# songlab-cal/CherryML

Hardware: AMD Instinct MI355X
Metric: cherry-pairs/sec (whole node) per EM iter (higher is better)
Workload: dtype f64

## Files before the change

cherryml_amd/csrc/eigh_planned.hip.h:

```cpp
#pragma once
#include "jacobi_block.hip.h"
#include "large_bank.hip.h"

enum {
  EC_STALL = 0,
  EC_FINAL = 1,
  EC_NSWEEP = 2,
  EC_MODE = 3,
  EC_SQ = 4,
  EC_ERR = 5,
  EC_ARRIVE = 6,
  EC_MASKED = 7,
  EC_SC = 8,
  EC_BANDS = 9,
  EC_SIGMA = 10,
  EC_TBSTALE = 11,
  EC_SKIP = 12,
  EC_REC = 16,
  EC_MAXREC = 12,
  EC_JSTATE = 64,
  EC_T0 = 80,
  EC_TSWEEP = 81,
  EC_TEND = 93,
  EC_NSTAMP = 95,
  EC_STAMPS = 96,
#ifdef CB_EIGH_STAMPS
  EC_WORDS = 96 + 96
#else
  EC_WORDS = 96
#endif
};
#ifdef CB_EIGH_STAMPS
__device__ __forceinline__ void lge_stamp(unsigned long long *ctl, int id) {
  if (blockIdx.x == 0 && blockIdx.y == 0 && threadIdx.x == 0) {
    const unsigned long long i = atomicAdd(ctl + EC_NSTAMP, 1ull);
    if (i < 96ull) ctl[EC_STAMPS + i] = ((unsigned long long)__builtin_amdgcn_s_memrealtime() << 8) | (unsigned long long)id;
  }
}
#define LGE_STAMP(ctl, id) lge_stamp(const_cast<unsigned long long *>(ctl), id)
#else

#define LGE_STAMP(ctl, id) ((void)0)
#endif
#define EC_NONE 0xFFFFFFFFull
#ifdef CB_PLAIN_WORDS
typedef const unsigned long long *lge_const_words;
#else
typedef const __attribute__((address_space(4))) unsigned long long *lge_const_words;
#endif

struct GramArgs {
  int LD, band, slot;
  int cap;
  int nsq;
  const double *G;
  double *X, *Xf;
  double *Gm, *dg;
  int so;
  unsigned long long *acc;
  unsigned long long *ctl;
  double trigger;
};

#define LGE_ACC_NT 32
#define LGE_ACC_COS 64
#define LGE_ACC_WORDS 128
#define LGE_ACC_UNIT 4503599627370496.0
__device__ __forceinline__ unsigned long long lge_fix(double x) {
  return x > 0.0 ? (unsigned long long)(fmin(x, 16.0) * LGE_ACC_UNIT) + 1ull : 0ull;
}

struct DecArgs {
  int on = 0;
  int cap = 0, nsq = 0, so = 0;
  double trigger = 0.0;
  const unsigned long long *acc = nullptr;
};

__device__ __forceinline__ double lge_lim(int order) {
  return order == 2 ? 1e-5 : order == 4 ? 2e-3 : order == 8 ? 0.06 : 0.5;
}

__global__ __launch_bounds__(512, 6) void lge_gram(GramArgs a) {
  __shared__ double sRed[8][256];
  __shared__ double sDg[2][32][16];
  __shared__ double sD[2][16];
  __shared__ double sStat[3][4];
  const unsigned long long *ctl = a.ctl;
  LGE_STAMP(ctl, 4);
  {
    lge_const_words cw = (lge_const_words)ctl;
    const unsigned long long w_stall = cw[EC_STALL], w_final = cw[EC_FINAL];
    if (w_stall != 0ull || (unsigned long long)a.slot > w_final) return;
  }
  const int LD = a.LD, nt = LD / 16;
  const int tm = blockIdx.x / nt, tn = blockIdx.x - tm * nt;
  const int m0 = tm * 16, n0 = tn * 16;
  const int wave = threadIdx.x >> 6, lane = threadIdx.x & 63, lo = lane & 15, hi = lane >> 4;
  const double *rowA = a.G + (size_t)(m0 + lo) * LD + 4 * hi, *rowB = a.G + (size_t)(n0 + lo) * LD + 4 * hi;
  d4 acc0 = {0.0, 0.0, 0.0, 0.0}, acc1 = acc0;
  double da = 0.0, db = 0.0;
  const int nchunks = LD / 16;
  for (int j0 = wave; j0 < nchunks; j0 += 32) {
    d4 av[4], bv[4];
#pragma unroll
    for (int u = 0; u < 4; ++u) {
      const int j = min(j0 + 8 * u, nchunks - 1);
      av[u] = *reinterpret_cast<const d4 *>(rowA + 16 * j);
      bv[u] = *reinterpret_cast<const d4 *>(rowB + 16 * j);
    }
#pragma unroll
    for (int u = 0; u < 4; ++u) {
      if (j0 + 8 * u < nchunks) {
        acc0 = mfma_f64(av[u][0], bv[u][0], acc0);
        acc1 = mfma_f64(av[u][1], bv[u][1], acc1);
        acc0 = mfma_f64(av[u][2], bv[u][2], acc0);
        acc1 = mfma_f64(av[u][3], bv[u][3], acc1);
        da += (av[u][0] * av[u][0] + av[u][1] * av[u][1]) + (av[u][2] * av[u][2] + av[u][3] * av[u][3]);
        db += (bv[u][0] * bv[u][0] + bv[u][1] * bv[u][1]) + (bv[u][2] * bv[u][2] + bv[u][3] * bv[u][3]);
      }
    }
  }
  const d4 acc = acc0 + acc1;
#pragma unroll
  for (int r = 0; r < 4; ++r) sRed[wave][r * 64 + lane] = acc[r];
  sDg[0][wave * 4 + hi][lo] = da;
  sDg[1][wave * 4 + hi][lo] = db;
  __syncthreads();
  if (threadIdx.x < 32) {
    const int w = threadIdx.x >> 4, c = threadIdx.x & 15;
    double s0 = 0.0, s1 = 0.0, s2 = 0.0, s3 = 0.0;
#pragma unroll
    for (int p = 0; p < 32; p += 4) {
      s0 += sDg[w][p][c];
      s1 += sDg[w][p + 1][c];
      s2 += sDg[w][p + 2][c];
      s3 += sDg[w][p + 3][c];
    }
    sD[w][c] = (s0 + s1) + (s2 + s3);
  }
  __syncthreads();
  double mc2 = 0.0;
  if (threadIdx.x < 256) {
    const int t = threadIdx.x, r = t >> 6, l = t & 63;
    const int ri = (l >> 4) + 4 * r, ci = l & 15;
    const int row = m0 + ri, col = n0 + ci;
    double g = 0.0;
#pragma unroll
    for (int w = 0; w < 8; ++w) g += sRed[w][t];
    const double gii = sD[0][ri], gjj = sD[1][ci];
    double x = 0.0;
    const double g2 = g * g, ab = gii * gjj;
    if (!(g2 == g2) || !(ab == ab)) mc2 = INFINITY;
    if (row != col && g2 > ab * (CB_JAC_SKIP * CB_JAC_SKIP)) {
      mc2 = fmax(mc2, g2 * fast_rcp(ab));
      const double d = gjj - gii;
      x = d != 0.0 ? 0.5 * atan(2.0 * g * fast_rcp(d)) : (g > 0.0 ? 0.78539816339744831 : -0.78539816339744831);
    }
    const int bd = row / JB_W - col / JB_W;
    const bool far = bd > a.band || -bd > a.band;
    a.X[(size_t)row * LD + col] = x;
    a.Xf[(size_t)row * LD + col] = far ? x : 0.0;
    if (a.so) {
      a.Gm[(size_t)row * LD + col] = g;
      if (row == col) a.dg[row] = gii;
    }
    double rs = fabs(x), rsf = far ? fabs(x) : 0.0;
#pragma unroll
    for (int m = 1; m < 16; m <<= 1) {
      rs += __shfl_xor(rs, m);
      rsf += __shfl_xor(rsf, m);
      mc2 = fmax(mc2, __shfl_xor(mc2, m));
    }
#pragma unroll
    for (int m = 16; m < 64; m <<= 1) {
      rs = fmax(rs, __shfl_xor(rs, m));
      rsf = fmax(rsf, __shfl_xor(rsf, m));
      mc2 = fmax(mc2, __shfl_xor(mc2, m));
    }
    if (l == 0) {
      sStat[0][r] = rs;
      sStat[1][r] = rsf;
      sStat[2][r] = mc2;
    }
  }
  __syncthreads();
  if (threadIdx.x < 3) {
    const int k = threadIdx.x;
    const double v = fmax(fmax(sStat[k][0], sStat[k][1]), fmax(sStat[k][2], sStat[k][3]));
    if (k < 2) atomicAdd(a.acc + k * LGE_ACC_NT + tm, lge_fix(v));
    else atomicMax(a.acc + LGE_ACC_COS + 16 * (blockIdx.x & 3), dbl_bits(v));
  }
}

struct LgeDecision {
  unsigned long long mode, sq, sc_bits;
};
struct LgeAcc {
  unsigned long long w = 0ull, c2 = 0ull;
};
__device__ __forceinline__ LgeAcc lge_acc_request(const DecArgs &d) {
  LgeAcc q;
  if (d.on) {
    q.w = d.acc[threadIdx.x & 63];
    lge_const_words ar = (lge_const_words)d.acc;
#pragma unroll
    for (int i = 0; i < 4; ++i) {
      const unsigned long long c = ar[LGE_ACC_COS + 16 * i];
      q.c2 = c > q.c2 ? c : q.c2;
    }
  }
  return q;
}
__device__ __forceinline__ double lge_uniform(double v, int lane) {
  return __hiloint2double(__builtin_amdgcn_readlane(__double2hiint(v), lane), __builtin_amdgcn_readlane(__double2loint(v), lane));
}
__device__ __forceinline__ LgeDecision lge_decide_here(int slot, const DecArgs &d, const LgeAcc &q, unsigned long long *ctl,
                                                       unsigned long long nsweep) {
  double v = (double)q.w * (1.0 / LGE_ACC_UNIT);
#pragma unroll
  for (int m = 1; m < 32; m <<= 1) v = fmax(v, __shfl_xor(v, m));
  const double rowsum = lge_uniform(v, 0), rowsum_far = lge_uniform(v, 32);
  double c2;
  memcpy(&c2, &q.c2, 8);
  LgeDecision o{0ull, 0ull, 0x3FF0000000000000ull};
  const bool bad = q.c2 >= 0x7FF0000000000000ull;
  bool masked = false, fin = false;
  if (!bad) {
    masked = c2 > d.trigger * d.trigger || rowsum > 1.0;
    const double rsu = masked ? rowsum_far : rowsum;
    const bool so = d.so != 0 && !masked && c2 > 1e-16 && rowsum <= 0.3;
    const double r2 = rowsum * rowsum;
    fin = !masked && (c2 <= 1e-16 || (so && c2 * r2 * r2 <= 4e-28));
    int order = rsu <= lge_lim(2) ? 2 : rsu <= lge_lim(4) ? 4 : rsu <= lge_lim(8) ? 8 : 12;
    if (order > d.cap) order = d.cap;
    const double lim = lge_lim(order);
    double sc = 1.0;
    while (rsu * sc > lim) {
      sc *= 0.5;
      ++o.sq;
    }
    unsigned long long damped = 0ull;
    if (o.sq > (unsigned long long)d.nsq) {
      o.sq = (unsigned long long)d.nsq;
      sc = lim / rsu;
      damped = 1ull;
    }
    o.sc_bits = dbl_bits(sc);
    o.mode = (unsigned long long)order | (masked ? 256ull : 0ull) | (damped << 9) | (so ? 1024ull : 0ull) | (1ull << 16);
  }
  if (blockIdx.x == 0 && blockIdx.y == 0 && threadIdx.x == 0) {
    const unsigned long long k = nsweep;
    ctl[EC_NSWEEP] = k + 1;
    if (bad) {
      ctl[EC_ERR] = 2ull;
      ctl[EC_STALL] = 1ull;
    }
    if (fin) ctl[EC_FINAL] = (unsigned long long)slot;
    ctl[EC_MASKED] = masked ? 1ull : 0ull;
    ctl[EC_MODE] = o.mode;
    ctl[EC_SQ] = o.sq;
    ctl[EC_SC] = o.sc_bits;
    if (k < EC_MAXREC) {
      ctl[EC_TSWEEP + k] = __builtin_amdgcn_s_memrealtime();
      ctl[EC_REC + 4 * k + 0] = dbl_bits(sqrt(c2));
      ctl[EC_REC + 4 * k + 1] = dbl_bits(rowsum);
      ctl[EC_REC + 4 * k + 2] = dbl_bits(rowsum_far);
      ctl[EC_REC + 4 * k + 3] = o.mode | (o.sq << 24) | ((unsigned long long)slot << 32);
    }
  }
  return o;
}

#ifdef CB_DECIDE_KERNEL
__global__ void lge_decide_k(int slot, DecArgs d, unsigned long long *ctl) {
  const LgeAcc q = lge_acc_request(d);
  lge_const_words cw = (lge_const_words)ctl;
  const unsigned long long w_stall = cw[EC_STALL], w_final = cw[EC_FINAL], w_nsw = cw[EC_NSWEEP];
  if (w_stall != 0ull || (unsigned long long)slot > w_final) return;
  (void)lge_decide_here(slot, d, q, ctl, w_nsw);
}
#endif

#ifdef CB_NANCHECK
__global__ void lge_residual(int LD, const double *A, const double *Ut, const double *lam, unsigned long long *ctl) {
  const int k = blockIdx.x;
  double m = 0.0;
  for (int i = threadIdx.x; i < LD; i += blockDim.x) {
    double r = -lam[k] * Ut[(size_t)k * LD + i];
    for (int j = 0; j < LD; ++j) r = fma(A[(size_t)i * LD + j], Ut[(size_t)k * LD + j], r);
    m = fmax(m, fabs(r));
    if (!(r == r)) m = INFINITY;
  }
  m = wave_max(m);
  if ((threadIdx.x & 63) == 0) atomicMax(ctl + 92, dbl_bits(m));
}
#endif
#ifdef CB_NANCHECK
__global__ void lge_orthcheck(int LD, const double *R, unsigned long long slot, unsigned long long *ctl) {
  lge_const_words cw = (lge_const_words)ctl;
  if (cw[EC_STALL] != 0ull || slot > cw[EC_FINAL] || !(cw[EC_MODE] >> 16)) return;
  const int k = blockIdx.x;
  double m = 0.0;
  for (int j = threadIdx.x; j < LD; j += blockDim.x) {
    double d = j == k ? -1.0 : 0.0;
    for (int i = 0; i < LD; ++i) d = fma(R[(size_t)i * LD + k], R[(size_t)i * LD + j], d);
    m = fmax(m, fabs(d));
    if (!(d == d)) m = INFINITY;
  }
  m = wave_max(m);
  if ((threadIdx.x & 63) == 0) {
    const unsigned long long old = atomicMax(ctl + 91, dbl_bits(m));
    if (dbl_bits(m) > old) ctl[90] = slot;
  }
}
#endif
#ifdef CB_NANCHECK
__global__ void lge_nancheck(int LD, const double *buf, unsigned long long tag, unsigned long long *ctl) {
  const size_t i = (size_t)blockIdx.x * blockDim.x + threadIdx.x;
  if (i >= (size_t)LD * LD) return;
  const double v = buf[i];
  if (!(v - v == 0.0)) atomicCAS(ctl + 94, 0ull, tag);
}
#endif

enum { EG_P2 = 0, EG_P34, EG_T1, EG_RP, EG_SQ, EG_GR, EG_R4 };

struct EgArgs {
  int LD, slot, kind, q;
  int cap;
  int early;
  const unsigned long long *ctl;
  const double *X, *Xf;
  double *P2, *P4;
  double *B0, *B1, *B2;
  double *T;
  double *R[2], *Rt[2];
  double *Rfin;
  const double *Gin;
  double *Gout;
  DecArgs dec;
  unsigned long long *zacc;
};


__device__ __forceinline__ double lge_ld(const double *base, int s, int LD, int c0, unsigned lane_bytes) {
  const __amdgpu_buffer_rsrc_t rs = __builtin_amdgcn_make_buffer_rsrc(const_cast<double *>(base), 0, 0x7fffffff, 0x00027000);
  return __builtin_bit_cast(double, __builtin_amdgcn_raw_buffer_load_b64(rs, (int)lane_bytes, (int)((unsigned)(4 * s * LD + c0) * 8u), 0));
}

__device__ __forceinline__ double lge_fold8(double (*sRed)[256], d4 acc, int wave, int lane, int et) {
  if (wave >= 4) {
#pragma unroll
    for (int r = 0; r < 4; ++r) sRed[wave - 4][r * 64 + lane] = acc[r];
  }
  __syncthreads();
  if (wave < 4) {
#pragma unroll
    for (int r = 0; r < 4; ++r) acc[r] += sRed[wave][r * 64 + lane];
  }
  __syncthreads();
  if (wave < 4) {
#pragma unroll
    for (int r = 0; r < 4; ++r) sRed[wave][r * 64 + lane] = acc[r];
  }
  __syncthreads();
  return (sRed[0][et] + sRed[1][et]) + (sRed[2][et] + sRed[3][et]);
}

#define LGE_UU 13
template <int KIND>
__global__ __launch_bounds__(512) void lge_gemm(EgArgs a) {
  __shared__ double sRed[4][256];
  const unsigned long long *ctl = a.ctl;
  LGE_STAMP(ctl, 10 + KIND);
  const int LD = a.LD, nt = LD / 16;
  const int tm = blockIdx.x / nt, tn = blockIdx.x - tm * nt;
  const int m0 = tm * 16, n0 = tn * 16;
  const int wave = __builtin_amdgcn_readfirstlane(threadIdx.x >> 6), lane = threadIdx.x & 63, lo = lane & 15, hi = lane >> 4;
  const int nsteps = LD / 4;
  const unsigned loff = (unsigned)(hi * LD + lo) * 8u;
  const int et = threadIdx.x & 255, er = et >> 6, el = et & 63;
  const int row = m0 + (el >> 4) + 4 * er, col = n0 + (el & 15);
  const size_t idx = (size_t)row * LD + col;
  const bool ep = threadIdx.x < 256;
  const double *Ap = nullptr, *Bp = nullptr, *Ep = nullptr;
  if (KIND == EG_T1) { Ap = a.P4; Bp = a.B2; Ep = a.B1; }
  if (KIND == EG_RP) { Ap = a.P4; Bp = a.T; Ep = a.B0; }
  if (KIND == EG_SQ) { Ap = a.Rt[a.q & 1]; Bp = a.R[a.q & 1]; }
  if (KIND == EG_GR) { Ap = a.Rfin; Bp = a.Gin; }
  if (KIND == EG_R4) { Ap = a.P2; Bp = a.B0; Ep = a.P2; }
  double av[LGE_UU], bv[LGE_UU], e1 = 0.0, ex = 0.0;
  const bool early = KIND != EG_P2 && a.early != 0;
  if (early) {
#pragma unroll
    for (int u = 0; u < LGE_UU; ++u) {
      const int sk = min(wave + 8 * u, nsteps - 1);
      av[u] = lge_ld(Ap, sk, LD, m0, loff);
      bv[u] = lge_ld(Bp, sk, LD, n0, loff);
    }
    if (Ep && ep) e1 = Ep[idx];
  }
  LgeAcc accq;
  if (KIND == EG_P2) accq = lge_acc_request(a.dec);
  lge_const_words cw = (lge_const_words)ctl;
  const unsigned long long w_stall = cw[EC_STALL], w_final = cw[EC_FINAL], w_nsw = cw[EC_NSWEEP];
  unsigned long long mode = cw[EC_MODE], w_sq = cw[EC_SQ], w_sc = cw[EC_SC];
  if (w_stall != 0ull || (unsigned long long)a.slot > w_final) return;
  if (KIND == EG_P2 && a.dec.on) {
    const LgeDecision dd = lge_decide_here(a.slot, a.dec, accq, const_cast<unsigned long long *>(ctl), w_nsw);
    mode = dd.mode;
    w_sq = dd.sq;
    w_sc = dd.sc_bits;
  }
  if (!(mode >> 16)) return;
  if (KIND == EG_GR && a.zacc && blockIdx.x == 0 && threadIdx.x < LGE_ACC_WORDS)
    a.zacc[threadIdx.x] = 0ull;
  const int order = (int)(mode & 255ull);
  const bool masked = (mode & (256ull | 1024ull)) != 0ull;
  const int sq = (int)w_sq;
  double sc;
  memcpy(&sc, &w_sc, 8);
  const double *Xu = masked ? a.Xf : a.X;
  if (KIND == EG_R4 && order != 4) return;
  if (KIND == EG_T1 && order != 12) return;
  if (KIND == EG_RP && order < 8) return;
  if (KIND == EG_SQ && a.q >= sq) return;
  if (!early) {
    const double *pa = KIND == EG_P2 ? Xu : Ap, *pb = KIND == EG_P2 ? Xu : Bp;
#pragma unroll
    for (int u = 0; u < LGE_UU; ++u) {
      const int sk = min(wave + 8 * u, nsteps - 1);
      av[u] = lge_ld(pa, sk, LD, m0, loff);
      bv[u] = lge_ld(pb, sk, LD, n0, loff);
    }
    if (KIND != EG_P2 && Ep && ep) e1 = Ep[idx];
  }
  if ((KIND == EG_P2 || KIND == EG_R4) && ep) ex = Xu[idx];
  d4 acc = {0.0, 0.0, 0.0, 0.0};
#pragma unroll
  for (int u = 0; u < LGE_UU; ++u)
    if (wave + 8 * u < nsteps) acc = mfma_f64(av[u], bv[u], acc);
  for (int s0 = wave + 8 * LGE_UU; s0 < nsteps; s0 += 8 * LGE_UU) {
    const double *pa = KIND == EG_P2 ? Xu : Ap, *pb = KIND == EG_P2 ? Xu : Bp;
#pragma unroll
    for (int u = 0; u < LGE_UU; ++u) {
      const int sk = min(s0 + 8 * u, nsteps - 1);
      av[u] = lge_ld(pa, sk, LD, m0, loff);
      bv[u] = lge_ld(pb, sk, LD, n0, loff);
    }
#pragma unroll
    for (int u = 0; u < LGE_UU; ++u)
      if (s0 + 8 * u < nsteps) acc = mfma_f64(av[u], bv[u], acc);
  }
  const double v = lge_fold8(sRed, acc, wave, lane, et);
  if (!ep) return;
  const double edl = row == col ? 1.0 : 0.0, s2 = sc * sc;
  if (KIND == EG_P2) {
    if (order == 2) {
      a.Rfin[idx] = fma(-0.5 * s2, v, fma(sc, ex, edl));
    } else {
      a.P2[idx] = v;
      if (a.cap == 4) a.B0[idx] = fma(-s2 * (1.0 / 24.0), v, (sc * (1.0 / 6.0)) * ex);
    }
  } else if (KIND == EG_R4) {
    a.Rfin[idx] = fma(-s2, v, fma(-0.5 * s2, e1, fma(sc, ex, edl)));
  } else if (KIND == EG_T1) {
    a.T[idx] = fma(s2 * s2, v, e1);
  } else if (KIND == EG_RP) {
    const double o = fma(s2 * s2, v, e1);
    if (sq == 0) a.Rfin[idx] = o;
    else {
      a.R[0][idx] = o;
      a.Rt[0][(size_t)col * LD + row] = o;
    }
  } else if (KIND == EG_SQ) {
    if (a.q == sq - 1) a.Rfin[idx] = v;
    else {
      a.R[(a.q + 1) & 1][idx] = v;
      a.Rt[(a.q + 1) & 1][(size_t)col * LD + row] = v;
    }
  } else {
    a.Gout[idx] = v;
  }
}

__global__ __launch_bounds__(512) void lge_p34(EgArgs a) {
  __shared__ double sRed[8][256];
  const unsigned long long *ctl = a.ctl;
  LGE_STAMP(ctl, 17);
  const int LD = a.LD, nt = LD / 16;
  const int tm = blockIdx.x / nt, tn = blockIdx.x - tm * nt;
  const int m0 = tm * 16, n0 = tn * 16;
  const int wave = __builtin_amdgcn_readfirstlane(threadIdx.x >> 6), lane = threadIdx.x & 63, lo = lane & 15, hi = lane >> 4;
  const int w4 = wave & 3;
  const bool fourth = wave >= 4;
  const int nsteps = LD / 4;
  const unsigned loff = (unsigned)(hi * LD + lo) * 8u;
  const int et = threadIdx.x & 255, er = et >> 6, el = et & 63;
  const int row = m0 + (el >> 4) + 4 * er, col = n0 + (el & 15);
  const size_t idx = (size_t)row * LD + col;
  const bool ep = threadIdx.x < 256;
  double av[LGE_UU], bv[LGE_UU], e2 = 0.0;
  const bool early = a.early != 0;
  if (early) {
#pragma unroll
    for (int u = 0; u < LGE_UU; ++u) {
      const int sk = min(w4 + 4 * u, nsteps - 1);
      bv[u] = lge_ld(a.P2, sk, LD, n0, loff);
      if (fourth) av[u] = lge_ld(a.P2, sk, LD, m0, loff);
    }
    if (ep) e2 = a.P2[idx];
  }
  lge_const_words cw = (lge_const_words)ctl;
  const unsigned long long w_stall = cw[EC_STALL], w_final = cw[EC_FINAL], mode = cw[EC_MODE], w_sc = cw[EC_SC];
  if (w_stall != 0ull || (unsigned long long)a.slot > w_final) return;
  if (!(mode >> 16)) return;
  const int order = (int)(mode & 255ull);
  if (order < 4) return;
  const bool masked = (mode & (256ull | 1024ull)) != 0ull;
  double sc;
  memcpy(&sc, &w_sc, 8);
  const double *Xu = masked ? a.Xf : a.X;
  const double *Ap = fourth ? a.P2 : Xu;
  if (!early) {
#pragma unroll
    for (int u = 0; u < LGE_UU; ++u) {
      const int sk = min(w4 + 4 * u, nsteps - 1);
      bv[u] = lge_ld(a.P2, sk, LD, n0, loff);
      av[u] = lge_ld(Ap, sk, LD, m0, loff);
    }
    if (ep) e2 = a.P2[idx];
  } else if (!fourth) {
#pragma unroll
    for (int u = 0; u < LGE_UU; ++u) av[u] = lge_ld(Xu, min(w4 + 4 * u, nsteps - 1), LD, m0, loff);
  }
  double ex = 0.0;
  if (ep) ex = Xu[idx];
  d4 acc = {0.0, 0.0, 0.0, 0.0};
#pragma unroll
  for (int u = 0; u < LGE_UU; ++u)
    if (w4 + 4 * u < nsteps) acc = mfma_f64(av[u], bv[u], acc);
  for (int s0 = w4 + 4 * LGE_UU; s0 < nsteps; s0 += 4 * LGE_UU) {
#pragma unroll
    for (int u = 0; u < LGE_UU; ++u) {
      const int sk = min(s0 + 4 * u, nsteps - 1);
// ... 277 lines not shown
```

cherryml_amd/csrc/eigh_planned_host.hip.h:

```cpp
#pragma once

struct EighRecord {
  bool stall = false;
  int err = 0, nsweep = 0, final_slot = -1;
  double sigma = 0.0;
  bool tb_stale = false;
  struct {
    double c, rs, rsf;
    int order, sq, slot;
    bool masked, damped;
  } sweep[EC_MAXREC];
};

#ifndef CB_PLANNED_BAND
#define CB_PLANNED_BAND 1
#endif
#ifndef CB_LEAD_INNER
#define CB_LEAD_INNER 2
#endif
static const int kPlannedBand = CB_PLANNED_BAND;

static void eigh_plan_default(EighPlan &p, int extra = 0) {
  p = EighPlan{};
  p.lead_band = 1;
// ... 33 lines not shown
  }
  p.slot[n] = EighSlot{4, 0, 0, 1, 0, 2, 0};
  p.lead_band = (r.sweep[0].masked && r.sweep[0].c > 1e-3) ? 1 : 0;
}

static void eigh_plan_continue(const EighRecord &r, EighPlan &p) {
  eigh_plan_default(p, 0);
  const bool masked = r.nsweep > 0 && r.sweep[std::min(r.nsweep, (int)EC_MAXREC) - 1].masked;
  p.lead_band = masked ? 1 : 0;
}

static bool eigh_planned_setup(cb_bank *h) {
  if (h->ectl) return true;
  if (h->planned_unavailable) return false;
  if (h->LD / 16 > LGE_ACC_NT) return false;
  h->planned_unavailable = true;
  const int LD = h->LD;
  void *q = nullptr;
  if (hipMalloc(&q, EC_WORDS * sizeof(unsigned long long)) != hipSuccess) return false;
  h->allocs.push_back(q);
  unsigned long long *ctl = static_cast<unsigned long long *>(q);
  if (hipMalloc(&q, ((size_t)2 * LGE_ACC_WORDS + LD) * sizeof(double)) != hipSuccess) return false;
  h->allocs.push_back(q);
  h->epart = static_cast<double *>(q);
  if (!h->epin) {
    if (hipHostMalloc(&q, 2 * (EC_WORDS + 16) * sizeof(unsigned long long), hipHostMallocCoherent | hipHostMallocMapped) != hipSuccess) {
      (void)hipGetLastError();
      return false;
    }
    memset(q, 0, 2 * (EC_WORDS + 16) * sizeof(unsigned long long));
    h->epin = static_cast<unsigned long long *>(q);
  }
  const int RS = LD + ((2 - LD % 32 + 32) % 32);
  const size_t lds = (size_t)(16 * RS + 3 * 16 * 17 + JB_WAVES * 256) * sizeof(double);
  if (hipFuncSetAttribute(reinterpret_cast<const void *>(lgj_round), hipFuncAttributeMaxDynamicSharedMemorySize, (int)lds) != hipSuccess)
    return false;
  if (hipMemsetAsync(ctl, 0, EC_WORDS * sizeof(unsigned long long), h->stream) != hipSuccess) return false;
  h->ectl = ctl;
  h->planned_unavailable = false;
  return true;
}

#ifdef CB_NANCHECK
#define NANCHECK(buf, tag) hipLaunchKernelGGL(lge_nancheck, dim3((unsigned)((LL + 255) / 256)), dim3(256), 0, h->stream, LD, buf, (unsigned long long)(tag), ctl)
#else
#define NANCHECK(buf, tag) ((void)0)
#endif
static int enqueue_planned_solve(cb_bank *h, const EighPlan &p, unsigned long long seq, int first_slot = 0, double tb_rho_max = 0.0,
                                 const TbTableArgs &tbt = TbTableArgs{}) {
  const int LD = h->LD, nt = LD / 16, nb = LD / JB_W;
  const size_t LL = (size_t)LD * LD;
  unsigned long long *ctl = h->ectl;
  unsigned long long *eacc = reinterpret_cast<unsigned long long *>(h->epart);
  double *Gb[2] = {h->Gc, h->Gc2};
  double *X = h->gx, *Xf = h->gx + LL, *P2 = h->gx + 2 * LL, *P3 = h->gx + 3 * LL, *P4 = h->gx + 4 * LL, *B0 = h->gx + 5 * LL,
         *B1 = h->gx + 6 * LL, *B2 = h->gx + 7 * LL, *T = h->gx + 8 * LL, *R0 = h->gx + 9 * LL, *R0t = h->gx + 10 * LL,
         *R1 = h->gx + 11 * LL, *R1t = h->gx + 6 * LL,
         *Rfin = h->gx + 3 * LL;
  const int RS = LD + ((2 - LD % 32 + 32) % 32);
  const size_t lds = (size_t)(16 * RS + 3 * 16 * 17 + JB_WAVES * 256) * sizeof(double);
  if (first_slot > 0) {
    hipLaunchKernelGGL(lge_resume, dim3(1), dim3(64), 0, h->stream, ctl);
  } else {
    if (!h->begin_folded) hipLaunchKernelGGL(lge_begin, dim3(1), dim3(256), 0, h->stream, LD, h->A, h->sigma, ctl, eacc);
    NANCHECK(h->U, 1);
    NANCHECK(h->A, 2);
    hipLaunchKernelGGL(lge_plain, dim3((unsigned)(nt * nt)), dim3(512), 0, h->stream, LD, h->U, h->A, h->Vc, h->sigma, Gb[0], nullptr);
  }
  unsigned long long *jstate = ctl + EC_JSTATE;
  int shift = 0;
  auto band_pass = [&](double *G, const unsigned long long *must_nonzero) {
    for (int w = 0; w < 2; ++w)
      hipLaunchKernelGGL(lgj_round, dim3(nb / 2), dim3(JB_THREADS), lds, h->stream, LD, ((shift + w) & 1) && nb > 2 ? -2 : -1,
                         must_nonzero ? 1 : CB_LEAD_INNER, G,
                         jstate, ctl + EC_STALL, must_nonzero);
    for (int k = 2; k <= kPlannedBand && k < nb; ++k)
      for (int par = 0; par < 2; ++par)
        hipLaunchKernelGGL(lgj_round, dim3((unsigned)(((nb + 2 * k - 1) / (2 * k)) * k)), dim3(JB_THREADS), lds, h->stream, LD,
                           -(10 + 2 * (k - 2) + par), 0, G, jstate, ctl + EC_STALL, must_nonzero);
    ++shift;
  };
  if (p.lead_band) band_pass(Gb[first_slot & 1], nullptr);
  const dim3 tiles((unsigned)(nt * nt));
  for (int i = 0; i < p.nslots; ++i) {
    const EighSlot &q = p.slot[i];
    const int s = first_slot + i;
    double *Gin = Gb[s & 1], *Gout = Gb[(s + 1) & 1];
    unsigned long long *acc = eacc + (size_t)(s & 1) * LGE_ACC_WORDS;
    GramArgs ga{LD, kPlannedBand, s, q.cap, q.cap == 12 ? q.nsq : 0, Gin, X, Xf, P3, h->epart + (size_t)2 * LGE_ACC_WORDS,
                q.so, acc, ctl, 3e-4};
    NANCHECK(Gin, 1000 + s * 100 + 1);
    hipLaunchKernelGGL(lge_gram, tiles, dim3(512), 0, h->stream, ga);
    NANCHECK(X, 1000 + s * 100 + 2);
    DecArgs dec;
    dec.on = 1; dec.cap = ga.cap; dec.nsq = ga.nsq; dec.so = q.so; dec.acc = acc; dec.trigger = ga.trigger;
#ifdef CB_DECIDE_KERNEL
    hipLaunchKernelGGL(lge_decide_k, dim3(1), dim3(64), 0, h->stream, s, dec, ctl);
    dec.on = 0;
#endif
    if (q.so) {
      SoArgs so{LD, s, ctl, ga.Gm, ga.dg, X, Xf, q.expect_run && i >= 1, dec};
#ifdef CB_NO_EARLY
      so.early = 0;
#endif
      hipLaunchKernelGGL(lge_so, tiles, dim3(512), 0, h->stream, so);
      NANCHECK(Xf, 1000 + s * 100 + 3);
    }
    EgArgs e{};
    if (!q.so) e.dec = dec;
    e.zacc = acc;
    e.LD = LD; e.slot = s; e.cap = q.cap; e.ctl = ctl; e.X = X; e.Xf = Xf; e.P2 = P2; e.P4 = P4; e.B0 = B0; e.B1 = B1; e.B2 = B2; e.T = T;
    e.R[0] = R0; e.R[1] = R1; e.Rt[0] = R0t; e.Rt[1] = R1t; e.Rfin = Rfin; e.Gin = Gin; e.Gout = Gout;
    auto gemm = [&](int kind, int qq = 0) {
      EgArgs c = e;
      c.kind = kind;
      c.q = qq;
      const int xo = q.expect_order;
      c.early = !q.expect_run ? 0 : kind == EG_P34 ? xo >= 4 : kind == EG_T1 ? xo == 12 : kind == EG_RP ? xo >= 8 :
                kind == EG_SQ ? qq < q.expect_sq : kind == EG_R4 ? xo == 4 : 1;
#ifdef CB_NO_EARLY
      c.early = 0;
#endif
      switch (kind) {
        case EG_P2: hipLaunchKernelGGL(lge_gemm<EG_P2>, tiles, dim3(512), 0, h->stream, c); break;
        case EG_P34: hipLaunchKernelGGL(lge_p34, tiles, dim3(512), 0, h->stream, c); break;
        case EG_T1: hipLaunchKernelGGL(lge_gemm<EG_T1>, tiles, dim3(512), 0, h->stream, c); break;
        case EG_RP: hipLaunchKernelGGL(lge_gemm<EG_RP>, tiles, dim3(512), 0, h->stream, c); break;
        case EG_SQ: hipLaunchKernelGGL(lge_gemm<EG_SQ>, tiles, dim3(512), 0, h->stream, c); break;
        case EG_R4: hipLaunchKernelGGL(lge_gemm<EG_R4>, tiles, dim3(512), 0, h->stream, c); break;
        default: hipLaunchKernelGGL(lge_gemm<EG_GR>, tiles, dim3(512), 0, h->stream, c); break;
      }
    };
    gemm(EG_P2);
    if (q.cap == 12) {
      gemm(EG_P34);
      gemm(EG_T1);
      gemm(EG_RP);
      for (int k = 0; k < q.nsq; ++k) gemm(EG_SQ, k);
    } else if (q.cap == 4) {
      gemm(EG_R4);
    }
    NANCHECK(Rfin, 1000 + s * 100 + 4);
#ifdef CB_NANCHECK
    hipLaunchKernelGGL(lge_orthcheck, dim3((unsigned)LD), dim3(256), 0, h->stream, LD, Rfin, (unsigned long long)s, ctl);
#endif
    gemm(EG_GR);
    NANCHECK(Gout, 1000 + s * 100 + 5);
    if (q.band_after) band_pass(Gout, ctl + EC_MASKED);
  }
  volatile unsigned long long *pin = h->epin + (size_t)(seq & 1ull) * (EC_WORDS + 16);
  hipLaunchKernelGGL(lge_norms, dim3((LD + 3) / 4), dim3(256), 0, h->stream, LD, Gb[0], Gb[1], h->X, ctl, pin, seq, h->sigma, tb_rho_max);
  LAUNCH_STOP(stop_event(h, EV_EIGH), lge_finish, dim3((LD + 3) / 4 + 1), dim3(256), 0, h->stream, LD, Gb[0], Gb[1], h->X, h->sigma, h->lam, h->U, h->Vc,
                     ctl, tbt, pin, seq);
#ifdef CB_NANCHECK
  hipLaunchKernelGGL(lge_residual, dim3((unsigned)LD), dim3(256), 0, h->stream, LD, h->A, h->Vc, h->lam, ctl);
#endif
  HIP_TRY(hipGetLastError());
  return CB_OK;
}

static int eigh_planned_record(cb_bank *h, unsigned long long seq, EighRecord &r) {
  volatile unsigned long long *pin = h->epin + (size_t)(seq & 1ull) * (EC_WORDS + 16);
  const auto t0 = std::chrono::steady_clock::now();
  bool got = false;
  for (unsigned it = 0;; ++it) {
    if (pin[EC_WORDS] == seq) {
      got = true;
      break;
    }
    if (it == 0) ++h->record_spins;
#if defined(__x86_64__)
    __builtin_ia32_pause();
#endif
    if ((it & 4095u) == 4095u && std::chrono::duration<double, std::milli>(std::chrono::steady_clock::now() - t0).count() > 200.0) break;
  }
  if (!got) {
    HIP_TRY(hipStreamSynchronize(h->stream));
    if (pin[EC_WORDS] != seq) return fail(CB_EHIP, "eigensolver: the record of the planned solve never reached the host");
  }
  std::atomic_thread_fence(std::memory_order_acquire);
  r = EighRecord{};
  r.stall = pin[EC_STALL] != 0ull;
  r.err = (int)pin[EC_ERR];
  {
    const unsigned long long ns = pin[EC_NSWEEP];
    r.nsweep = (int)(ns < (unsigned long long)EC_MAXREC ? ns : (unsigned long long)EC_MAXREC);
  }
  r.final_slot = pin[EC_FINAL] == EC_NONE ? -1 : (int)pin[EC_FINAL];
  {
    const unsigned long long sb = pin[EC_SIGMA];
    memcpy(&r.sigma, &sb, 8);
  }
  r.tb_stale = pin[EC_TBSTALE] != 0ull;
  for (int k = 0; k < r.nsweep; ++k) {
    unsigned long long w[4] = {pin[EC_REC + 4 * k], pin[EC_REC + 4 * k + 1], pin[EC_REC + 4 * k + 2], pin[EC_REC + 4 * k + 3]};
    memcpy(&r.sweep[k].c, &w[0], 8);
    memcpy(&r.sweep[k].rs, &w[1], 8);
    memcpy(&r.sweep[k].rsf, &w[2], 8);
    r.sweep[k].order = (int)(w[3] & 255ull);
    r.sweep[k].masked = (w[3] & 256ull) != 0ull;
    r.sweep[k].damped = (w[3] & 512ull) != 0ull;
    r.sweep[k].sq = (int)((w[3] >> 24) & 255ull);
    r.sweep[k].slot = (int)(w[3] >> 32);
  }
  if (getenv("CB_DEBUG")) {
    fprintf(stderr, "[cherrybank] planned eigh %llu:%s", seq, r.stall ? " STALL" : "");
    for (int k = 0; k < r.nsweep; ++k)
// ... 40 lines not shown
```

cherryml_amd/csrc/handle_host.hip.h:

```cpp
#pragma once
#include <hip/hip_ext.h>
#include <future>
struct EighSlot {
  int cap = 12;
  int nsq = 0;
  int band_after = 0;
  int so = 0;
  int expect_run = 1, expect_order = 12, expect_sq = 2;
};
struct EighPlan {
  int lead_band = 1;
  int nslots = 0;
  EighSlot slot[EC_MAXREC];
};
struct cb_bank {
  int dev = 0, S = 0, L = 0, B = 0;
  int B_cap = 0;
  hipStream_t xstream[3] = {};
  hipEvent_t ev_fork = nullptr, ev_join[3] = {};
  int tr_epochs = 0;
  uint64_t tr_sig = 0;
  int last_form = 0;
  double tr_pow_b1 = 1.0, tr_pow_b2 = 1.0;
  int dtype = CB_F64;
  int LD = 0;
  bool large = false;
  hipStream_t own_stream = nullptr, stream = nullptr;
  std::vector<void *> allocs;
  std::vector<double> n_host;
  double *t = nullptr;
  double *Ct = nullptr;
  double *n_dev = nullptr;
  double *inv_n = nullptr;
  double *ones = nullptr;
  double *Cq = nullptr;
  int nq = 0;
  double *dirsum = nullptr;
  double *dirsum_g = nullptr;
  int Bl = 0;
  double *t_live = nullptr;
  int *nlive = nullptr;
  std::vector<int> nlive_host;
  double *Q = nullptr, *pi = nullptr, *loss = nullptr, *dQ = nullptr;
  int *status = nullptr;
  double *Gc2 = nullptr, *gx = nullptr;
  int last_light = 0;
  void *comm = nullptr;
  int (*allreduce)(const void *, void *, size_t, int, int, void *, hipStream_t) = nullptr;
  double *inv_n_global = nullptr;
  std::vector<double> n_global;
  bool expm_only = false;
  bool per_bucket_products = false;
  bool sym_counts = false;
  int spec_sweeps = 0;
  double *A = nullptr, *dsq = nullptr, *Gc = nullptr, *Vc = nullptr, *U = nullptr, *lam = nullptr,
         *sigma = nullptr, *F = nullptr, *E = nullptr, *H = nullptr, *Gt = nullptr, *T = nullptr,
         *Mt_part = nullptr, *Mt = nullptr, *X = nullptr, *loss_part = nullptr;
  float *Ct32 = nullptr, *Gt32 = nullptr, *T32 = nullptr, *Uf = nullptr, *Utf = nullptr, *Af = nullptr, *Ff = nullptr;
  unsigned long long *off_bits = nullptr;
  unsigned long long *poll = nullptr;
  unsigned long long poll_seq = 0;
  unsigned long long *ectl = nullptr, *epin = nullptr;
  double *epart = nullptr;
  bool begin_folded = false;
  double *sigma_home = nullptr;
  double *sigma2 = nullptr;
  unsigned long long eseq = 0;
  bool planned_unavailable = false;
  int planned_solves = 0, planned_stalls = 0;
  long long record_spins = 0;
  std::vector<double> epoch_seconds;
  EighPlan eplan;
  int k3_chunk = 0, k3_nchunks = 0;
  double *Yk = nullptr, *Lk = nullptr;
  double phi_delta = 0.0;
  unsigned int *bank_queue = nullptr;
  unsigned char *bank_args = nullptr;
  int bank_slots = 0;
  int bank_claims = 0;
  bool bank_fused = false;
  int bank_kg = 1;
  bool bank_accum = false;
  CbTimeBasisHost tb;
  int tb_set = 0;
  double *tb_Ls[2] = {}, *tb_Lg[2] = {}, *tb_tf[2] = {}, *tb_tg[2] = {};
  std::future<CbTimeBasisHost> tb_next;
  bool tb_next_pending = false;
  int tb_next_epoch = 0;
  size_t tb_ew_lds[4] = {0, 0, 0, 0};
  int tb_builds = 0, tb_stale_epochs = 0;
  bool tb_failed = false;
  bool tb_block = false;
  bool bank_tb = false;
  int last_sweeps = 0;
  double *gn_scratch = nullptr, *gn_partial = nullptr;
  int gn_nw = 0;
  struct {
    double *Qn = nullptr, *QT = nullptr, *colsum = nullptr, *alpha = nullptr, *R = nullptr, *RT = nullptr, *E = nullptr,
           *ET = nullptr, *G = nullptr, *GT = nullptr, *Xbar = nullptr, *lpart = nullptr;
    int *nsq = nullptr;
    int cap_slots = 0;
  } gl;
  std::vector<double> t_host, t_live_host;
  bool have_prev = false;
  double *ws_ptr[16] = {};
  size_t ws_cap[16] = {};
  char *pin = nullptr;
  size_t pin_cap = 0, pin_off = 0;
  bool profile = false;
  int profile_every = 1;
  bool profile_now = false;
  hipEvent_t ev[CB_T_COUNT + 1] = {};
  bool ev_rec[CB_T_COUNT + 1] = {};
  double t_sum[CB_T_COUNT] = {};
  int t_calls = 0;
  bool t_pending = false;
  hipEvent_t ev2[CB_T_COUNT + 1] = {};
  bool ev_rec2[CB_T_COUNT + 1] = {};
  bool t_pending2 = false;
};

static void swap_event_sets(cb_bank *h) {
  for (int i = 0; i <= CB_T_COUNT; ++i) {
    std::swap(h->ev[i], h->ev2[i]);
    std::swap(h->ev_rec[i], h->ev_rec2[i]);
  }
  std::swap(h->t_pending, h->t_pending2);
}

static void fold_pending(cb_bank *h);
enum { EV_START = 0, EV_EIGH, EV_K1, EV_K2, EV_K3, EV_K4, EV_SMALL, EV_END, EV_AR };
static void mark(cb_bank *h, int which) {
  if (!h->profile || !h->profile_now) return;
  if (!h->ev[which]) (void)hipEventCreate(&h->ev[which]);
  (void)hipEventRecord(h->ev[which], h->stream);
  h->ev_rec[which] = true;
}

static hipEvent_t stop_event(cb_bank *h, int which) {
  if (!h->profile || !h->profile_now) return nullptr;
  if (!h->ev[which] && hipEventCreate(&h->ev[which]) != hipSuccess) return nullptr;
  h->ev_rec[which] = true;
  return h->ev[which];
}
static void clear_marks(cb_bank *h) {
  if (h->profile && !h->profile_now) return;
// ... 77 lines not shown
```

cherryml_amd/csrc/train_host.hip.h:

```cpp
#pragma once
template <int NW>
static int launch_train_nw(cb_bank *h, const TrainArgs &a) {
  static_assert(NW == 4, "25 .. 32 states: the four-wave form only (see the kernels' launch bounds)");
  const size_t lds = (SmallLds<NW>::TOTAL + 72) * sizeof(double);
  if (h->S <= 24) return fail(CB_EINVAL, "internal: %d states dispatched to the one-kernel trainer", h->S);
  auto kern = small_train_kernel<2, 8, NW>;
  HIP_TRY(hipFuncSetAttribute(reinterpret_cast<const void *>(kern), hipFuncAttributeMaxDynamicSharedMemorySize, (int)lds));
  hipLaunchKernelGGL(kern, dim3(h->L), dim3(NW * 64), lds, h->stream, a);
  HIP_TRY(hipGetLastError());
  return CB_OK;
}

__global__ void tr_stamp(double *out) { *out = (double)__builtin_amdgcn_s_memrealtime(); }

static void set_epoch_seconds(cb_bank *h, const char *ticks, int E, double t_first_s) {
  h->epoch_seconds.assign((size_t)std::max(E, 0), 0.0);
  if (!ticks || E <= 0) return;
  std::vector<double> tk((size_t)E + 1);
  memcpy(tk.data(), ticks, ((size_t)E + 1) * sizeof(double));
  for (int e = 0; e < E; ++e) h->epoch_seconds[e] = t_first_s + (tk[e] - tk[E]) * 1e-8;
}

static int run_fused_training_large(cb_bank *h, double *pi_param, double *up_param, const double *mask, int E,
                                    double lr, int do_adam, int flags, double *loss_curve, double *Q_best,
// ... 22 lines not shown
    const int head[3] = {mask ? 1 : 0, do_adam ? 1 : 0, (flags & CB_NORMALIZE) ? 1 : 0};
    mix(head, sizeof head);
    mix(&lr, sizeof lr);
    if (mask) mix(mask, SS * sizeof(double));
    if (sig == 0) sig = 1;
  }
  if (resume && (h->tr_epochs <= 0 || h->tr_sig != sig))
    return fail(CB_EINVAL, "CB_TRAIN_RESUME: no finished training call with the same mask / optimiser / learning rate / "
                           "normalisation on this handle");
  if (resume && Q_pow2) return fail(CB_EINVAL, "CB_TRAIN_RESUME: Q_pow2 must be NULL");
  const int e0 = resume ? h->tr_epochs : 0;
  int slot = 0;
  auto alloc = [&](double **p, size_t n) -> bool { return ws_get(h, slot++, n, p); };
  auto release = [&]() {
    (void)hipStreamSynchronize(h->stream);
    if (h->sigma_home) h->sigma = h->sigma_home;
    h->begin_folded = false;
    h->profile_now = h->profile;
  };
  double *d_pi = nullptr, *d_up = nullptr, *d_mom = nullptr, *d_mask = nullptr, *d_loss = nullptr, *d_Qb = nullptr,
         *d_Ql = nullptr, *d_Qp = nullptr, *d_vec = nullptr, *d_time = nullptr;
  const size_t nmom = 2 * (S + nup);
  auto at = [&](int s, double **p, size_t n) -> bool { return ws_get(h, s, n, p); };
  bool ok = at(0, &d_pi, S) && at(1, &d_up, nup) && at(2, &d_mom, nmom) && at(3, &d_loss, E) && at(4, &d_Qb, SS) &&
            at(5, &d_Ql, SS) && (!mask || at(6, &d_mask, SS)) &&
            (!(Q_pow2 && n_pow2 > 0) || at(7, &d_Qp, std::max<size_t>(n_pow2, 16) * SS)) && at(8, &d_vec, (size_t)LD + S + 8) &&
            at(9, &d_time, (size_t)E + 1);
  (void)alloc;
  if (!ok) {
    release();
    return fail(CB_ENOMEM, "fused training: device allocation failed");
  }
  if (dbg) fprintf(stderr, "[cherrybank] large trainer: workspaces ready after %.2f ms\n", now() - t_enter);
  int rc = CB_OK;
#define TRYH(expr) \
  if (rc == CB_OK && (expr) != hipSuccess) rc = fail(CB_EHIP, "%s failed", #expr)
  {
    const size_t up_bytes = (S + nup + SS + 64) * sizeof(double);
    const size_t down_bytes = (S + nup + 2 * (size_t)E + 16 + (2 + (size_t)(d_Qp ? n_pow2 : 0)) * SS + 64) * sizeof(double);
    if (!pin_reserve(h, std::max(up_bytes, down_bytes) + 1024)) {
      release();
      return fail(CB_ENOMEM, "fused training: pinned staging allocation failed");
    }
  }
  if (!resume) {
    TRYH(h2d_staged(h, d_pi, pi_param, S * sizeof(double)));
    TRYH(h2d_staged(h, d_up, up_param, nup * sizeof(double)));
    TRYH(hipMemsetAsync(d_mom, 0, nmom * sizeof(double), h->stream));
    TRYH(hipMemsetAsync(d_Qb, 0, SS * sizeof(double), h->stream));
    TRYH(hipMemsetAsync(d_Ql, 0, SS * sizeof(double), h->stream));
  }
  if (mask && !resume) TRYH(h2d_staged(h, d_mask, mask, SS * sizeof(double)));
  const double init_state[2] = {INFINITY, INFINITY};
  LargeTrain a{};
  a.S = S; a.LD = LD; a.do_adam = do_adam; a.n_pow2 = d_Qp ? n_pow2 : 0;
  a.epoch0 = e0;
  a.p_pi = d_pi; a.p_up = d_up;
  a.m_pi = d_mom; a.v_pi = d_mom + S; a.m_up = d_mom + 2 * (size_t)S; a.v_up = a.m_up + nup;
  a.mask = d_mask; a.lr = lr; a.beta1 = 0.9; a.beta2 = 0.999; a.eps = 1e-8;
  a.pi = d_vec; a.gd = d_vec + LD; a.state = d_vec + LD + S;
  a.dsq = h->dsq; a.A = h->A; a.G = h->Mt; a.loss = h->loss;
  a.dirsum = h->comm ? h->dirsum_g : h->dirsum;
  a.inv_n = (flags & CB_NORMALIZE) ? 1.0 / (h->comm ? h->n_global[0] : h->n_host[0]) : 1.0;
  a.loss_curve = d_loss; a.time_curve = d_time; a.Q_last = d_Ql; a.Q_best = d_Qb; a.Q_pow2 = d_Qp;
  if (dbg) fprintf(stderr, "[cherrybank] large trainer: copies enqueued after %.2f ms\n", now() - t_enter);
  if (!resume) TRYH(h2d_staged(h, a.state, init_state, sizeof init_state));
  TRYH(hipStreamSynchronize(h->stream));
  if (dbg) fprintf(stderr, "[cherrybank] large trainer: synced after %.2f ms\n", now() - t_enter);
  if (h->profile) fold_pending(h);
  if (dbg) fprintf(stderr, "[cherrybank] large trainer: parameters uploaded after %.2f ms\n", now() - t_enter);
  double pow_b1 = resume ? h->tr_pow_b1 : 1.0, pow_b2 = resume ? h->tr_pow_b2 : 1.0;
  if (!h->sigma2) {
    if (dev_alloc(h, &h->sigma2, 2) != CB_OK) {
      release();
      return CB_ENOMEM;
    }
  }
  if (!h->sigma_home) h->sigma_home = h->sigma;
  TRYH(hipMemsetAsync(h->sigma2, 0, 2 * sizeof(double), h->stream));
  h->last_form = 4000;
  h->tr_epochs = 0;
  const int fault_epoch = cb_test_hook("CB_FAULT_INJECT") ? atoi(cb_test_hook("CB_FAULT_INJECT")) : -1000;
  const bool planned = !cb_test_hook("CB_EIGH_HOST") && !cb_test_hook("CB_NO_HYBRID") && LD % 16 == 0 && LD / JB_W >= 8 && eigh_planned_setup(h);
  EighPlan &plan = h->eplan;
  if (!resume) eigh_plan_default(plan);
  if (!resume) {
    tb_drop_next(h);
    h->tb = CbTimeBasisHost{};
    h->tb_failed = false;
  }
  const int short_plans = cb_test_hook("CB_EIGH_SHORT_PLAN") ? std::max(1, atoi(cb_test_hook("CB_EIGH_SHORT_PLAN"))) : 0;
  auto shorten = [&]() {
    if (!short_plans) return;
    plan.nslots = 1;
    if (short_plans >= 2) plan.slot[0] = EighSlot{2, 0, plan.slot[0].band_after, 0};
  };
  shorten();
  const double trace_slow = getenv("CB_TRACE_SLOW") ? atof(getenv("CB_TRACE_SLOW")) : 0.0;
  const double t_first_s = (now() - t_enter) * 1e-3;
  hipLaunchKernelGGL(tr_stamp, dim3(1), dim3(1), 0, h->stream, d_time + E);
  for (int e = 0; e < E && rc == CB_OK; ++e) {
    const double te0 = trace_slow > 0.0 ? now() : 0.0;
    double te_fold = 0.0, te_enq = 0.0, te_rec = 0.0;
    h->profile_now = h->profile && (e0 + e) % h->profile_every == 0;
    if (h->profile_now) {
      swap_event_sets(h);
      fold_pending(h);
    }
    if (trace_slow > 0.0) te_fold = now();
    clear_marks(h);
    const bool use_plan = planned && h->have_prev && e0 + e >= 3;
    {
      const int par = (e0 + e) & 1;
      h->sigma = h->sigma2 + par;
      a.sig_cur = reinterpret_cast<unsigned long long *>(h->sigma2 + par);
      a.sig_next = reinterpret_cast<unsigned long long *>(h->sigma2 + (par ^ 1));
      a.ectl = use_plan ? h->ectl : nullptr;
      a.eacc = use_plan ? reinterpret_cast<unsigned long long *>(h->epart) : nullptr;
      h->begin_folded = use_plan;
    }
    LAUNCH_STOP(stop_event(h, EV_START), lt_build, dim3(LD), dim3(256), 0, h->stream, a, e0 + e);
    rc = large_eval(h, flags & CB_NORMALIZE, h->loss, h->Mt, true, nullptr, false, use_plan ? &plan : nullptr);
    h->begin_folded = false;
    if (trace_slow > 0.0) te_enq = now();
    if (rc == CB_OK && use_plan) {
      EighRecord rec;
      rc = eigh_planned_record(h, h->eseq, rec);
      ++h->planned_solves;
      if (rc == CB_OK && rec.err == 2) rc = fail(CB_ENUMERIC, "eigensolver: non-finite input");
      int slots_done = plan.nslots;
      for (int attempt = 0; rc == CB_OK && rec.stall && attempt < 3; ++attempt) {
        ++h->planned_stalls;
        EighPlan more;
        eigh_plan_continue(rec, more);
        clear_marks(h);
        mark(h, EV_START);
        rc = large_eval(h, flags & CB_NORMALIZE, h->loss, h->Mt, true, nullptr, false, &more, slots_done);
        slots_done += more.nslots;
        if (rc == CB_OK) rc = eigh_planned_record(h, h->eseq, rec);
        if (rc == CB_OK && rec.err == 2) rc = fail(CB_ENUMERIC, "eigensolver: non-finite input");
      }
      bool host_solved = false;
      if (rc == CB_OK && rec.stall) {
        host_solved = true;
        if (hipStreamSynchronize(h->stream) != hipSuccess) rc = fail(CB_EHIP, "hipStreamSynchronize failed (host-driven solver fallback)");
        else if (hipMemsetAsync(h->ectl, 0, sizeof(unsigned long long), h->stream) != hipSuccess)
          rc = fail(CB_EHIP, "hipMemsetAsync failed (host-driven solver fallback)");
        clear_marks(h);
        mark(h, EV_START);
        if (rc == CB_OK) rc = large_eval(h, flags & CB_NORMALIZE, h->loss, h->Mt, true, nullptr);
      }
      if (rc == CB_OK && !host_solved && h->bank_tb) {
        if (rec.tb_stale) {
          clear_marks(h);
          mark(h, EV_START);
          h->tb_block = true;
          rc = large_eval(h, flags & CB_NORMALIZE, h->loss, h->Mt, true, nullptr, true, nullptr);
          h->tb_block = false;
        }
        if (rc == CB_OK) rc = tb_maintain(h, h->Bl, e0 + e, 2.0 * rec.sigma, rec.tb_stale);
        if (rc == CB_OK && rec.tb_stale) ++h->tb_stale_epochs;
      }
      if (rc == CB_OK) {
        const EighPlan prev = plan;
        eigh_plan_from_record(rec, prev, plan);
        shorten();
// ... 317 lines not shown
```

Before: 1.543 billion.

## Exploit symmetry: compute upper-triangular tiles in Gram and P2 GEMM, mirror outputs

Result: faster. 1.581 billion (median of 5 runs) (+2.5%).

```diff
diff --git a/cherryml_amd/csrc/eigh_planned.hip.h b/cherryml_amd/csrc/eigh_planned.hip.h
--- a/cherryml_amd/csrc/eigh_planned.hip.h
+++ b/cherryml_amd/csrc/eigh_planned.hip.h
@@ -60,7 +60,18 @@
   unsigned long long *acc;
   unsigned long long *ctl;
   double trigger;
+  int tri;
 };
+
+__device__ __forceinline__ void lge_tri_tile(int b, int nt, int &tm, int &tn) {
+  const int w = 2 * nt + 1;
+  int r = (int)(0.5f * ((float)w - sqrtf((float)(w * w - 8 * b))));
+  r = max(0, min(r, nt - 1));
+  while (r > 0 && r * (w - r) / 2 > b) --r;
+  while ((r + 1) * (w - r - 1) / 2 <= b) ++r;
+  tm = __builtin_amdgcn_readfirstlane(r);
+  tn = __builtin_amdgcn_readfirstlane(r + b - r * (w - r) / 2);
+}
 
 #define LGE_ACC_NT 32
 #define LGE_ACC_COS 64
@@ -85,7 +96,9 @@
   __shared__ double sRed[8][256];
   __shared__ double sDg[2][32][16];
   __shared__ double sD[2][16];
-  __shared__ double sStat[3][4];
+  __shared__ double sStat[5][4];
+  double(*sT)[16 * 17] = reinterpret_cast<double(*)[16 * 17]>(&sDg[0][0][0]);
+  static_assert(sizeof(sDg) >= 2 * 16 * 17 * sizeof(double), "the transposed tile lives in sDg");
   const unsigned long long *ctl = a.ctl;
   LGE_STAMP(ctl, 4);
   {
@@ -94,9 +107,11 @@
     if (w_stall != 0ull || (unsigned long long)a.slot > w_final) return;
   }
   const int LD = a.LD, nt = LD / 16;
-  const int tm = blockIdx.x / nt, tn = blockIdx.x - tm * nt;
+  int tm = blockIdx.x / nt, tn = blockIdx.x - tm * nt;
+  if (a.tri) lge_tri_tile((int)blockIdx.x, nt, tm, tn);
+  const bool mir = a.tri != 0 && tm < tn;
   const int m0 = tm * 16, n0 = tn * 16;
-  const int wave = threadIdx.x >> 6, lane = threadIdx.x & 63, lo = lane & 15, hi = lane >> 4;
+  const int wave = __builtin_amdgcn_readfirstlane(threadIdx.x >> 6), lane = threadIdx.x & 63, lo = lane & 15, hi = lane >> 4;
   const double *rowA = a.G + (size_t)(m0 + lo) * LD + 4 * hi, *rowB = a.G + (size_t)(n0 + lo) * LD + 4 * hi;
   d4 acc0 = {0.0, 0.0, 0.0, 0.0}, acc1 = acc0;
   double da = 0.0, db = 0.0;
@@ -149,13 +164,18 @@
 #pragma unroll
     for (int w = 0; w < 8; ++w) g += sRed[w][t];
     const double gii = sD[0][ri], gjj = sD[1][ci];
-    double x = 0.0;
+    double x = 0.0, xm = 0.0;
     const double g2 = g * g, ab = gii * gjj;
     if (!(g2 == g2) || !(ab == ab)) mc2 = INFINITY;
     if (row != col && g2 > ab * (CB_JAC_SKIP * CB_JAC_SKIP)) {
       mc2 = fmax(mc2, g2 * fast_rcp(ab));
       const double d = gjj - gii;
       x = d != 0.0 ? 0.5 * atan(2.0 * g * fast_rcp(d)) : (g > 0.0 ? 0.78539816339744831 : -0.78539816339744831);
+      xm = d != 0.0 ? -x : x;
+    }
+    if (mir) {
+      sT[0][ri * 17 + ci] = xm;
+      sT[1][ri * 17 + ci] = g;
     }
     const int bd = row / JB_W - col / JB_W;
     const bool far = bd > a.band || -bd > a.band;
@@ -190,6 +210,39 @@
     const double v = fmax(fmax(sStat[k][0], sStat[k][1]), fmax(sStat[k][2], sStat[k][3]));
     if (k < 2) atomicAdd(a.acc + k * LGE_ACC_NT + tm, lge_fix(v));
     else atomicMax(a.acc + LGE_ACC_COS + 16 * (blockIdx.x & 3), dbl_bits(v));
+  }
+  if (!mir) return;
+  if (threadIdx.x < 256) {
+    const int t = threadIdx.x, r = t >> 6, l = t & 63;
+    const int ri = (l >> 4) + 4 * r, ci = l & 15;
+    const int row = n0 + ri, col = m0 + ci;
+    const double x = sT[0][ci * 17 + ri];
+    const int bd = row / JB_W - col / JB_W;
+    const bool far = bd > a.band || -bd > a.band;
+    a.X[(size_t)row * LD + col] = x;
+    a.Xf[(size_t)row * LD + col] = far ? x : 0.0;
+    if (a.so) a.Gm[(size_t)row * LD + col] = sT[1][ci * 17 + ri];
+    double rs = fabs(x), rsf = far ? fabs(x) : 0.0;
+#pragma unroll
+    for (int m = 1; m < 16; m <<= 1) {
+      rs += __shfl_xor(rs, m);
+      rsf += __shfl_xor(rsf, m);
+    }
+#pragma unroll
+    for (int m = 16; m < 64; m <<= 1) {
+      rs = fmax(rs, __shfl_xor(rs, m));
+      rsf = fmax(rsf, __shfl_xor(rsf, m));
+    }
+    if (l == 0) {
+      sStat[3][r] = rs;
+      sStat[4][r] = rsf;
+    }
+  }
+  __syncthreads();
+  if (threadIdx.x < 2) {
+    const int k = threadIdx.x;
+    const double v = fmax(fmax(sStat[3 + k][0], sStat[3 + k][1]), fmax(sStat[3 + k][2], sStat[3 + k][3]));
+    atomicAdd(a.acc + k * LGE_ACC_NT + tn, lge_fix(v));
   }
 }
 
@@ -341,6 +394,7 @@
   double *Gout;
   DecArgs dec;
   unsigned long long *zacc;
+  int tri;
 };
 
 
@@ -372,10 +426,13 @@
 template <int KIND>
 __global__ __launch_bounds__(512) void lge_gemm(EgArgs a) {
   __shared__ double sRed[4][256];
+  __shared__ double sT[KIND == EG_P2 ? 16 * 17 : 1];
   const unsigned long long *ctl = a.ctl;
   LGE_STAMP(ctl, 10 + KIND);
   const int LD = a.LD, nt = LD / 16;
-  const int tm = blockIdx.x / nt, tn = blockIdx.x - tm * nt;
+  int tm = blockIdx.x / nt, tn = blockIdx.x - tm * nt;
+  if (KIND == EG_P2 && a.tri) lge_tri_tile((int)blockIdx.x, nt, tm, tn);
+  const bool mir = KIND == EG_P2 && a.tri != 0 && tm < tn;
   const int m0 = tm * 16, n0 = tn * 16;
   const int wave = __builtin_amdgcn_readfirstlane(threadIdx.x >> 6), lane = threadIdx.x & 63, lo = lane & 15, hi = lane >> 4;
   const int nsteps = LD / 4;
@@ -383,6 +440,7 @@
   const int et = threadIdx.x & 255, er = et >> 6, el = et & 63;
   const int row = m0 + (el >> 4) + 4 * er, col = n0 + (el & 15);
   const size_t idx = (size_t)row * LD + col;
+  const size_t idm = (size_t)(n0 + (el >> 4) + 4 * er) * LD + m0 + (el & 15);
   const bool ep = threadIdx.x < 256;
   const double *Ap = nullptr, *Bp = nullptr, *Ep = nullptr;
   if (KIND == EG_T1) { Ap = a.P4; Bp = a.B2; Ep = a.B1; }
@@ -390,7 +448,7 @@
   if (KIND == EG_SQ) { Ap = a.Rt[a.q & 1]; Bp = a.R[a.q & 1]; }
   if (KIND == EG_GR) { Ap = a.Rfin; Bp = a.Gin; }
   if (KIND == EG_R4) { Ap = a.P2; Bp = a.B0; Ep = a.P2; }
-  double av[LGE_UU], bv[LGE_UU], e1 = 0.0, ex = 0.0;
+  double av[LGE_UU], bv[LGE_UU], e1 = 0.0, ex = 0.0, exm = 0.0;
   const bool early = KIND != EG_P2 && a.early != 0;
   if (early) {
 #pragma unroll
@@ -437,6 +495,7 @@
     if (KIND != EG_P2 && Ep && ep) e1 = Ep[idx];
   }
   if ((KIND == EG_P2 || KIND == EG_R4) && ep) ex = Xu[idx];
+  if (KIND == EG_P2 && mir && ep) exm = Xu[idm];
   d4 acc = {0.0, 0.0, 0.0, 0.0};
 #pragma unroll
   for (int u = 0; u < LGE_UU; ++u)
@@ -454,14 +513,27 @@
       if (s0 + 8 * u < nsteps) acc = mfma_f64(av[u], bv[u], acc);
   }
   const double v = lge_fold8(sRed, acc, wave, lane, et);
-  if (!ep) return;
+  if (!ep && !mir) return;
   const double edl = row == col ? 1.0 : 0.0, s2 = sc * sc;
   if (KIND == EG_P2) {
+    if (ep) {
+      if (order == 2) {
+        a.Rfin[idx] = fma(-0.5 * s2, v, fma(sc, ex, edl));
+      } else {
+        a.P2[idx] = v;
+        if (a.cap == 4) a.B0[idx] = fma(-s2 * (1.0 / 24.0), v, (sc * (1.0 / 6.0)) * ex);
+      }
+    }
+    if (!mir) return;
+    if (ep) sT[((el >> 4) + 4 * er) * 17 + (el & 15)] = v;
+    __syncthreads();
+    if (!ep) return;
+    const double vm = sT[(el & 15) * 17 + (el >> 4) + 4 * er];
     if (order == 2) {
-      a.Rfin[idx] = fma(-0.5 * s2, v, fma(sc, ex, edl));
+      a.Rfin[idm] = fma(-0.5 * s2, vm, fma(sc, exm, 0.0));
     } else {
-      a.P2[idx] = v;
-      if (a.cap == 4) a.B0[idx] = fma(-s2 * (1.0 / 24.0), v, (sc * (1.0 / 6.0)) * ex);
+      a.P2[idm] = vm;
+      if (a.cap == 4) a.B0[idm] = fma(-s2 * (1.0 / 24.0), vm, (sc * (1.0 / 6.0)) * exm);
     }
   } else if (KIND == EG_R4) {
     a.Rfin[idx] = fma(-s2, v, fma(-0.5 * s2, e1, fma(sc, ex, edl)));
diff --git a/cherryml_amd/csrc/eigh_planned_host.hip.h b/cherryml_amd/csrc/eigh_planned_host.hip.h
--- a/cherryml_amd/csrc/eigh_planned_host.hip.h
+++ b/cherryml_amd/csrc/eigh_planned_host.hip.h
@@ -139,15 +139,17 @@
   };
   if (p.lead_band) band_pass(Gb[first_slot & 1], nullptr);
   const dim3 tiles((unsigned)(nt * nt));
+  const int tri = h->eigh_full_tiles ? 0 : 1;
+  const dim3 sym_tiles((unsigned)(tri ? nt * (nt + 1) / 2 : nt * nt));
   for (int i = 0; i < p.nslots; ++i) {
     const EighSlot &q = p.slot[i];
     const int s = first_slot + i;
     double *Gin = Gb[s & 1], *Gout = Gb[(s + 1) & 1];
     unsigned long long *acc = eacc + (size_t)(s & 1) * LGE_ACC_WORDS;
     GramArgs ga{LD, kPlannedBand, s, q.cap, q.cap == 12 ? q.nsq : 0, Gin, X, Xf, P3, h->epart + (size_t)2 * LGE_ACC_WORDS,
-                q.so, acc, ctl, 3e-4};
+                q.so, acc, ctl, 3e-4, tri};
     NANCHECK(Gin, 1000 + s * 100 + 1);
-    hipLaunchKernelGGL(lge_gram, tiles, dim3(512), 0, h->stream, ga);
+    hipLaunchKernelGGL(lge_gram, sym_tiles, dim3(512), 0, h->stream, ga);
     NANCHECK(X, 1000 + s * 100 + 2);
     DecArgs dec;
     dec.on = 1; dec.cap = ga.cap; dec.nsq = ga.nsq; dec.so = q.so; dec.acc = acc; dec.trigger = ga.trigger;
@@ -172,6 +174,7 @@
       EgArgs c = e;
       c.kind = kind;
       c.q = qq;
+      c.tri = kind == EG_P2 ? tri : 0;
       const int xo = q.expect_order;
       c.early = !q.expect_run ? 0 : kind == EG_P34 ? xo >= 4 : kind == EG_T1 ? xo == 12 : kind == EG_RP ? xo >= 8 :
                 kind == EG_SQ ? qq < q.expect_sq : kind == EG_R4 ? xo == 4 : 1;
@@ -179,7 +182,7 @@
       c.early = 0;
 #endif
       switch (kind) {
-        case EG_P2: hipLaunchKernelGGL(lge_gemm<EG_P2>, tiles, dim3(512), 0, h->stream, c); break;
+        case EG_P2: hipLaunchKernelGGL(lge_gemm<EG_P2>, sym_tiles, dim3(512), 0, h->stream, c); break;
         case EG_P34: hipLaunchKernelGGL(lge_p34, tiles, dim3(512), 0, h->stream, c); break;
         case EG_T1: hipLaunchKernelGGL(lge_gemm<EG_T1>, tiles, dim3(512), 0, h->stream, c); break;
         case EG_RP: hipLaunchKernelGGL(lge_gemm<EG_RP>, tiles, dim3(512), 0, h->stream, c); break;
diff --git a/cherryml_amd/csrc/handle_host.hip.h b/cherryml_amd/csrc/handle_host.hip.h
--- a/cherryml_amd/csrc/handle_host.hip.h
+++ b/cherryml_amd/csrc/handle_host.hip.h
@@ -62,6 +62,7 @@
   unsigned long long poll_seq = 0;
   unsigned long long *ectl = nullptr, *epin = nullptr;
   double *epart = nullptr;
+  bool eigh_full_tiles = false;
   bool begin_folded = false;
   double *sigma_home = nullptr;
   double *sigma2 = nullptr;
diff --git a/cherryml_amd/csrc/train_host.hip.h b/cherryml_amd/csrc/train_host.hip.h
--- a/cherryml_amd/csrc/train_host.hip.h
+++ b/cherryml_amd/csrc/train_host.hip.h
@@ -128,6 +128,7 @@
   h->tr_epochs = 0;
   const int fault_epoch = cb_test_hook("CB_FAULT_INJECT") ? atoi(cb_test_hook("CB_FAULT_INJECT")) : -1000;
   const bool planned = !cb_test_hook("CB_EIGH_HOST") && !cb_test_hook("CB_NO_HYBRID") && LD % 16 == 0 && LD / JB_W >= 8 && eigh_planned_setup(h);
+  h->eigh_full_tiles = cb_test_hook("CB_EIGH_FULL_TILES") != nullptr;
   EighPlan &plan = h->eplan;
   if (!resume) eigh_plan_default(plan);
   if (!resume) {
```
